# n7koirala/image_matching

Hardware: AMD Instinct MI355X
Metric: encrypted DB vectors matched/sec (HyDia indexScenario, CKKS N=2^15) (higher is better)
Workload: dtype u64

## Files before the change

### image_matching_amd/csrc/context.cpp

```cpp
#include <algorithm>
#include <cmath>
#include <cstdio>
#include <cstdlib>
#include <cstring>

#include <sys/stat.h>

#include "hydia_core.h"

namespace hydia {

u64 mulmod_u64(u64 a, u64 b, u64 q) { return (u64)(((u128)a * b) % q); }
u64 powmod_u64(u64 a, u64 e, u64 q) {
    u64 r = 1 % q;
    a %= q;
    for (; e; e >>= 1) {
        if (e & 1) r = mulmod_u64(r, a, q);
        a = mulmod_u64(a, a, q);
    }
    return r;
}
u64 invmod_u64(u64 a, u64 q) { return powmod_u64(a % q, q - 2, q); }

static bool miller_rabin(u64 n) {
// ... 292 lines not shown
                ifr[2 * i] = (double)itw[i];
                ifr[2 * i + 1] = (double)itw[i] / qd;
            }
        HIP_CHECK(hipMalloc((void **)&d_twf, 2 * tb));
        HIP_CHECK(hipMalloc((void **)&d_itwf, 2 * tb));
        HIP_CHECK(hipMemcpy(d_twf, fr.data(), 2 * tb, hipMemcpyHostToDevice));
        HIP_CHECK(hipMemcpy(d_itwf, ifr.data(), 2 * tb, hipMemcpyHostToDevice));
        std::vector<double> dr((size_t)nT * N), idr((size_t)nT * N);
        for (size_t i = 0; i < (size_t)nT * N; i++) {
            dr[i] = (double)tw[i];
            idr[i] = (double)itw[i];
        }
        HIP_CHECK(hipMalloc((void **)&d_twd, tb));
        HIP_CHECK(hipMalloc((void **)&d_itwd, tb));
        HIP_CHECK(hipMemcpy(d_twd, dr.data(), tb, hipMemcpyHostToDevice));
        HIP_CHECK(hipMemcpy(d_itwd, idr.data(), tb, hipMemcpyHostToDevice));
    }
    tabs = NttTables{d_tw, d_tw_sh, d_itw, d_itw_sh, d_mod, (const ulonglong2 *)d_twp, (const ulonglong2 *)d_itwp,
                     (const ulonglong2 *)d_twf, (const ulonglong2 *)d_itwf, (const double *)d_twd, (const double *)d_itwd, 0u};
    if (getenv("HYDIA_NTT_INT")) tabs.twf = tabs.itwf = nullptr;
    getenv_int_arith = getenv("HYDIA_NTT_INT") != nullptr;
    tabs.fp_mask = 0;
    for (int m = 0; m < nT; m++)
        if (tabs.twf != nullptr && mod[m].ks + 2 <= 47) tabs.fp_mask |= 1u << m;
    {
        const char *sw = getenv("HYDIA_NTT_1PASS");
        tabs.one_pass = !sw ? 0 : (sw[0] == 'p' ? 2 : 1);
        const char *mn = getenv("HYDIA_NTT_1PASS_MIN");
        tabs.one_pass_min = mn ? atoi(mn) : 1024;
        tabs.two_ip_launches = getenv("HYDIA_RELIN_TWO_IP_LAUNCHES") ? 1 : 0;
        tabs.no_drop_in_ip = getenv("HYDIA_NO_DROP_IN_IP") ? 1 : 0;
        tabs.int_epilogue = getenv("HYDIA_INT_EPILOGUE") ? 1 : 0;
        const char *g = getenv("HYDIA_IP_GROUP");
        tabs.ip_group = g && atoi(g) > 0 ? atoi(g) : 8;
        tabs.generic = getenv("HYDIA_NTT_GENERIC") ? 1 : 0;
        tabs.cf_wide = getenv("HYDIA_COLFUSE_WIDE") ? 1 : 0;
        tabs.p2_wg_sync = getenv("HYDIA_P2_WG_SYNC") ? 1 : 0;
        tabs.no_tw_lds = getenv("HYDIA_NO_TW_LDS") ? 1 : 0;
    }
    modup_per_digit = getenv("HYDIA_MODUP_PER_DIGIT") != nullptr;
    loop_a_separate_ip = getenv("HYDIA_LOOPA_SEPARATE_IP") != nullptr;
    loop_a_int_ip = getenv("HYDIA_LOOPA_INT_IP") != nullptr;
    loop_a_limb_fastest = getenv("HYDIA_LOOPA_LIMB_FASTEST") != nullptr;
    relin_separate_intt = getenv("HYDIA_RELIN_SEPARATE_INTT") != nullptr;
    tabs.pm_mask = 0;
    if (!getenv("HYDIA_NTT_INT") && !getenv("HYDIA_NTT_NO_PM"))
        for (int m = 0; m < nT; m++)
            if (!((tabs.fp_mask >> m) & 1u) && mod[m].q < (1ull << 60) && (1ull << 60) - mod[m].q < (1ull << 24)) tabs.pm_mask |= 1u << m;
    if (const char *e = getenv("HYDIA_TENSOR_BPP")) tensor_bpp = std::max(1, atoi(e));
    if (const char *e = getenv("HYDIA_TENSOR_NW")) tensor_nw = atoi(e);
    merge_rescale = getenv("HYDIA_NO_MERGE_RESCALE") == nullptr;
    fuse_ip = getenv("HYDIA_NO_FUSE_IP") == nullptr;
    fork_products = getenv("HYDIA_NO_FORK") == nullptr;
    fuse_loop_a = getenv("HYDIA_NO_FUSE_LOOPA") == nullptr;
    colfuse = getenv("HYDIA_NO_COLFUSE") == nullptr;
    if (const char *e = getenv("HYDIA_MATVEC")) {
        if (e[0] == 'h') matvec_mode = 1;
        else if (e[0] == 'b') matvec_mode = bsgs_babies();
        else if (e[0] >= '1' && e[0] <= '9') matvec_mode = babies_for(1, atoi(e));
        else matvec_mode = 0;
    }
    rot_packed = getenv("HYDIA_KEYS_UNPACKED") == nullptr;
    db_packed = getenv("HYDIA_DB_UNPACKED") == nullptr;
    db_seq_ok = getenv("HYDIA_DB_CT_MAJOR") == nullptr;
    for (int j = 1; j < nQ; j++)
        if (q[j] >> 48) db_packed = false;
    HIP_CHECK(hipMalloc((void **)&d_rotptrs, sizeof(u64 *) * (size_t)p.dim));
    HIP_CHECK(hipMalloc((void **)&d_rotgalois, sizeof(unsigned) * (size_t)p.dim));
    HIP_CHECK(hipMalloc((void **)&d_rotginv, sizeof(unsigned) * (size_t)p.dim));

}

Context::~Context() {
    (void)hipSetDevice(device);
    for (auto st : lane_stream) (void)hipStreamSynchronize(st);
    stream = lane_stream.empty() ? stream : lane_stream[0];
    for (auto &kv : timers)
        for (auto &ev : kv.second.pending) {
            (void)hipEventDestroy(ev.first);
            (void)hipEventDestroy(ev.second);
        }
    pool.trim();
    for (auto &kv : modup_plans)
        if (kv.second.d_tabs) (void)hipFree(kv.second.d_tabs);
    for (auto &kv : cf_plans)
        if (kv.second.dev) (void)hipFree(kv.second.dev);
    rot_keys[0] = relin_key;
    for (auto &kv : rot_keys)
        if (!kv.second.borrowed)
            for (void *p : {(void *)kv.second.d, (void *)kv.second.d_cell, (void *)kv.second.d_gal})
                if (p) (void)hipFree(p);
    if (keys_borrowed) d_rotpack = nullptr, d_sk = nullptr, d_pk = nullptr;
    for (void *p : {(void *)d_mod, (void *)d_tw, (void *)d_tw_sh, (void *)d_itw, (void *)d_itw_sh, (void *)d_twp, (void *)d_itwp, (void *)d_twf, (void *)d_itwf, (void *)d_twd, (void *)d_itwd,
                    (void *)d_rotptrs, (void *)d_rotpack, (void *)d_giant_keys, (void *)d_giant_gal, (void *)d_giant_ginv,
                    (void *)d_rotgalois, (void *)d_rotginv, (void *)d_sk, (void *)d_pk, (void *)d_db, (void *)d_rot_group, (void *)d_ksi})
        if (p) (void)hipFree(p);
    for (auto e : lane_ev) (void)hipEventDestroy(e);
    for (auto e : par_ev)
        if (e) (void)hipEventDestroy(e);
    for (size_t k = 1; k < lane_stream.size(); k++) (void)hipStreamDestroy(lane_stream[k]);
    if (stream) (void)hipStreamDestroy(stream);
}
void Context::set_lane(int k) {
    stream = lane_stream[k];
    pool.cur = k;
}
void Context::sync_all() {
    for (auto st : lane_stream) HIP_CHECK(hipStreamSynchronize(st));
}

LimbSel Context::sel_q(int nl) const { return sel_range(0, nl); }
LimbSel Context::sel_range(int lo, int hi) const {
    LimbSel s{};
    s.n = hi - lo;
    for (int j = lo; j < hi; j++) s.mod[j - lo] = j;
    return s;
}
LimbSel Context::sel_ext(int nl) const {
    LimbSel s{};
    s.n = nl + nP;
    for (int j = 0; j < nl; j++) s.mod[j] = j;
    for (int k = 0; k < nP; k++) s.mod[nl + k] = nQ + k;
    return s;
}
ScaleSel Context::scale_ninv(const LimbSel &s) const {
    ScaleSel r{};
    for (int i = 0; i < s.n; i++) {
        r.s[i] = mod[s.mod[i]].ninv;
        r.s_sh[i] = mod[s.mod[i]].ninv_sh;
    }
    return r;
}
ScaleSel Context::scale_of(const LimbSel &s, const std::vector<u64> &v, bool times_ninv) const {
    ScaleSel r{};
    for (int i = 0; i < s.n; i++) {
        u64 qq = q[s.mod[i]];
        u64 val = v[i] % qq;
        if (times_ninv) val = mulmod_u64(val, mod[s.mod[i]].ninv, qq);
        r.s[i] = val;
        r.s_sh[i] = shoup(val, qq);
    }
    return r;
}
u64 Context::galois_elt(int rot) const {
    u64 M = 2ull * N, g = 1;
    int r = ((rot % slots) + slots) % slots;
    for (int i = 0; i < r; i++) g = (g * 5) % M;
    return g;
}

void Context::adopt_keys(Context &src) {
    if (&src == this) return;
    if (src.device != device) throw std::runtime_error("hydia: keys can only be shared between contexts on the same GPU");
    if (src.nT != nT || src.N != N || src.prm.dnum != prm.dnum || src.prm.dim != prm.dim || src.q != q)
        throw std::runtime_error("hydia: keys can only be shared between contexts with identical parameters");
    if (relin_key.d || !rot_keys.empty() || d_sk || d_pk) throw StateError("hydia: this context already holds keys of its own");
    src.build_rotptrs();
    src.sync_all();
// ... 273 lines not shown
```

### image_matching_amd/csrc/evaluator.cpp

```cpp
#include <algorithm>
#include <cmath>
#include <cstring>

#include "hydia_core.h"

#include <exception>

namespace hydia {

static u64 shoup_h(u64 w, u64 q) { return (u64)(((u128)w << 64) / q); }

static void op_bytes(const char *op, size_t N, double transforms, double other_bytes) {
    hk::ledger_add(op, transforms * 2.0 * (double)N * 8.0 + other_bytes);
}

void Context::ntt_fwd(u64 *base, size_t outer, int X, const LimbSel &s) {
    if (X <= 0 || s.n <= 0) return;
    hk::ntt_forward(stream, tabs, prm.logN, base, base, outer, outer, X, s);
}
void Context::ntt_inv(const u64 *src, u64 *dst, size_t so, size_t dso, int X, const LimbSel &s, const ScaleSel &sc) {
    if (X <= 0 || s.n <= 0) return;
    hk::ntt_inverse(stream, tabs, prm.logN, src, dst, so, dso, X, s, sc);
}

// ... 127 lines not shown
    cf.usc = mod[l].ninv;
    cf.usc_sh = mod[l].ninv_sh;
    for (int k = 0; k < nP; k++) {
        const u64 qq = q[nQ + k];
        cf.smod[k] = nQ + k;
        cf.srow[k] = 1 + k;
        cf.ssc[k] = mulmod_u64(Phat_inv[k] % qq, mod[nQ + k].ninv, qq);
        cf.ssc_sh[k] = shoup_h(cf.ssc[k], qq);
        for (int j = 0; j < nl; j++) {
            u64 f = mulmod_u64(Phat_mod_q[k][j], Pinv_mod_q[j], q[j]);
            if (dbl) f = (f + f) % q[j];
            if (j < l) cf.f[k][j] = f;
            else cf.fl[k] = f;
        }
    }
    for (int j = 0; j < l; j++) {
        cf.tmod[j] = j;
        cf.trow[j] = j;
    }
    return cf_plan_store(key, std::move(maps));
}

const Context::CfPlan &Context::cf_plan_rescale(int nl) {
    const std::string key = "rs:" + std::to_string(nl);
    auto it = cf_plans.find(key);
    if (it != cf_plans.end()) return it->second;
    const int l = nl - 1;
    if (l > HY_CF_TGT) throw std::runtime_error("hydia: too many targets for the column-fused conversion");
    std::vector<ColFuse> maps(1);
    ColFuse &cf = maps[0];
    cf = ColFuse{};
    cf.nk = 0;
    cf.nt = l;
    cf.mdr = 1;
    cf.l = l;
    cf.umod = l;
    cf.urow = 0;
    cf.usc = mod[l].ninv;
    cf.usc_sh = mod[l].ninv_sh;
    for (int j = 0; j < l; j++) {
        cf.tmod[j] = j;
        cf.trow[j] = j;
    }
    return cf_plan_store(key, std::move(maps));
}

void Context::modup_digits(const u64 *c, size_t c_outer, int X, int nl, u64 *dig, bool copy_own, bool p1_only, const ProdSrc *ps, u64 *d2_out) {
    if (ps && !cf_ok()) throw std::runtime_error("hydia: fused product outside the column-fused pipeline");
    const int nE = nl + nP, nd = (nl + alpha - 1) / alpha;
    const size_t dig_x = (size_t)nd * nE * N;
    const LimbSel esel = sel_ext(nl), qsel = sel_q(nl);
    const ModUpPlan &pl = modup_plan(nl);
    u64 *y = pool.get((size_t)X * nl * N * sizeof(u64));
    if (cf_ok()) {
        const CfPlan &cp = cf_plan_modup(nl);
        const bool small = hk::ntt15_colfuse_small(X, nd);
        if (ps) {
            hk::ntt15_inverse_p2_prod(stream, tabs, *ps, y, (size_t)nl * N, X, qsel, d2_out);
            if (small) hk::ntt15_inverse_p1(stream, tabs, y, (size_t)nl * N, X, qsel, scale_of(qsel, pl.inv, true));
        } else if (small) {
            ntt_inv(c, y, c_outer, (size_t)nl * N, X, qsel, scale_of(qsel, pl.inv, true));
        } else {
            hk::ntt15_inverse_p2(stream, tabs, c, y, c_outer, (size_t)nl * N, X, qsel);
        }
        hk::ntt15_colfuse(stream, tabs, y, (size_t)nl * N, dig, dig_x, X, cp.dev, cp.host.data(), nd, small);
        pool.put(y);
        if (!p1_only) {
            if ((size_t)X * nd * nE < 128) {
                hk::ntt15_forward_p2(stream, tabs, dig, (size_t)nE * N, X * nd, esel);
            } else {
                for (int d = 0; d < nd; d++) {
                    const int lo = d * alpha, hi = std::min(lo + alpha, nl);
                    u64 *out = dig + (size_t)d * nE * N;
                    LimbSel rest{};
                    rest.n = nE - hi;
                    for (int t = hi; t < nE; t++) rest.mod[t - hi] = esel.mod[t];
                    if (lo > 0) hk::ntt15_forward_p2(stream, tabs, out, dig_x, X, sel_range(0, lo));
                    if (rest.n > 0) hk::ntt15_forward_p2(stream, tabs, out + (size_t)hi * N, dig_x, X, rest);
                }
            }
        }
        if (copy_own)
            for (int d = 0; d < nd; d++) {
                const int lo = d * alpha, hi = std::min(lo + alpha, nl);
                hk::copy_limbs(stream, N, c + (size_t)lo * N, dig + (size_t)d * nE * N + (size_t)lo * N, c_outer, dig_x, X, hi - lo);
            }
        return;
    }
    ntt_inv(c, y, c_outer, (size_t)nl * N, X, qsel, scale_of(qsel, pl.inv, true));
    hk::base_convert_digits(stream, d_mod, N, y, (size_t)nl * N, dig, dig_x, X, pl.d_tabs, nd, nl, nE, esel);
    const bool merged = !modup_per_digit && nd > 1 && (size_t)X * nd * nE < 128;
    if (merged) {
        if (p1_only) hk::ntt15_forward_p1(stream, tabs, dig, dig, (size_t)nE * N, (size_t)nE * N, X * nd, esel);
        else ntt_fwd(dig, (size_t)nE * N, X * nd, esel);
    }
    for (int d = 0; d < nd; d++) {
        const int lo = d * alpha, hi = std::min(lo + alpha, nl), sz = hi - lo;
        u64 *out = dig + (size_t)d * nE * N;
        LimbSel rest{};
        rest.n = nE - hi;
        for (int t = hi; t < nE; t++) rest.mod[t - hi] = esel.mod[t];
        if (!merged) {
            if (p1_only) {
                if (lo > 0) hk::ntt15_forward_p1(stream, tabs, out, out, dig_x, dig_x, X, sel_range(0, lo));
                if (rest.n > 0) hk::ntt15_forward_p1(stream, tabs, out + (size_t)hi * N, out + (size_t)hi * N, dig_x, dig_x, X, rest);
            } else {
                if (lo > 0) ntt_fwd(out, dig_x, X, sel_range(0, lo));
                ntt_fwd(out + (size_t)hi * N, dig_x, X, rest);
            }
        }
        if (copy_own) hk::copy_limbs(stream, N, c + (size_t)lo * N, out + (size_t)lo * N, c_outer, dig_x, X, sz);
    }
    pool.put(y);
}

void Context::ks_apply(const u64 *dig, size_t dig_x_stride, int X, int nl, const u64 *const *d_keys, int same_key,
                       const u64 *addend, size_t add_x_stride, size_t add_poly_stride, int add_polys,
// ... 203 lines not shown
    pool.put(y);
    std::vector<u64> pinv(Pinv_mod_q.begin(), Pinv_mod_q.begin() + nl);
    NttStore stp{};
    stp.mode = 1;
    stp.out = out;
    stp.nl = nl;
    stp.in = acc;
    stp.in_ls = nE;
    stp.mul = scale_of(qsel, pinv, false);
    stp.addend = addend;
    stp.add_x = add_x;
    stp.add_p = add_p;
    stp.add_polys = add_polys;
    stp.dbl = dbl ? 1 : 0;
    stp.ginv = d_ginv;
    stp.same_g = same_g;
    hk::ntt15_forward_p2_fused(stream, tabs, conv, (size_t)nl * N, XP, qsel, stp);
    pool.put(conv);
    pool.put(acc);
}

void Context::relinearize(Ct &c, bool dbl) {
    if (c.npoly != 3) return;
    if (!relin_key.d) throw StateError("hydia: relinearisation key not loaded");
    const int nl = c.nl, nE = nl + nP, nd = (nl + alpha - 1) / alpha, X = c.X;
    op_bytes("op:relinearize", N, (double)X * (nd * nE + 2 * nP + 2 * nl), (double)nd * 2 * nE * N * 8);
    if (ks_fused_ok()) {
        Ct out(this, X, 2, nl, c.scale);
        ks_fused(c.d + 2 * c.poly_elems(), c.ct_elems(), X, nl, relin_key.d, relin_key.d_cell, nullptr, c.d, c.ct_elems(), c.poly_elems(), 2, nullptr, 0, dbl,
                 out.d);
        c = std::move(out);
        return;
    }
    u64 *dig = pool.get((size_t)X * nd * nE * N * sizeof(u64));
    modup_digits(c.d + 2 * c.poly_elems(), c.ct_elems(), X, nl, dig);
    Ct out(this, X, 2, nl, c.scale);
    ks_apply(dig, (size_t)nd * nE * N, X, nl, relin_key.d_cell, 1, c.d, c.ct_elems(), c.poly_elems(), 2, nullptr, nullptr, 0, dbl,
             out.d);
    pool.put(dig);
    c = std::move(out);
}
void Context::rescale(Ct &c, const Ct *sub, const double *addc) {
    const int nl = c.nl, l = nl - 1, XP = c.X * c.npoly;
    if (nl < 2) throw std::runtime_error("hydia: rescale with one limb left");
    if (sub && (sub->X != c.X || sub->npoly != c.npoly || sub->nl < l)) throw std::runtime_error("hydia: rescale sub operand shape");
    op_bytes("op:rescale", N, (double)XP * nl, 0);
    u64 *t = pool.get((size_t)XP * N * sizeof(u64));
    const LimbSel last = sel_range(l, l + 1);
    u64 *tmp = pool.get((size_t)XP * l * N * sizeof(u64));
    const LimbSel qsel = sel_q(l);
    Ct out(this, c.X, c.npoly, l, c.scale / (double)q[l]);
    std::vector<u64> qi(ql_inv[l].begin(), ql_inv[l].begin() + l);
    const bool rcf = rescale_cf && cf_ok() && l <= HY_LC_LIMBS && l <= HY_CF_TGT && (q[l] >> 50) == 0 && XP >= 256;
    if (rcf) {
        hk::ntt15_inverse_p2(stream, tabs, c.d + (size_t)l * N, t, c.poly_elems(), (size_t)N, XP, last);
        const CfPlan &cp = cf_plan_rescale(nl);
        hk::ntt15_colfuse(stream, tabs, t, (size_t)N, tmp, (size_t)l * N, XP, cp.dev, cp.host.data(), 1, false);
        NttStore stp{};
        stp.mode = 2;
        stp.out = out.d;
        stp.nl = l;
        stp.in = c.d;
        stp.in_ls = c.lstride;
        stp.mul = scale_of(qsel, qi, false);
        stp.sub = sub ? sub->d : nullptr;
        stp.sub_ls = sub ? sub->lstride : 0;
        stp.has_addc = addc ? 1 : 0;
        stp.npoly = c.npoly;
        if (addc)
            for (int j = 0; j < l; j++) stp.addc[j] = double_to_mod(*addc * out.scale, q[j]);
        hk::ntt15_forward_p2_fused(stream, tabs, tmp, (size_t)l * N, XP, qsel, stp);
        pool.put(tmp);
        pool.put(t);
        c = std::move(out);
        return;
    }
    ntt_inv(c.d + (size_t)l * N, t, c.poly_elems(), (size_t)N, XP, last, scale_ninv(last));
    if (prm.logN == 15 && l <= HY_LC_LIMBS) {
        NttLoad ld{};
        ld.mode = 2;
        ld.y = t;
        ld.y_outer = (size_t)N;
        ld.l = l;
        NttStore stp{};
        stp.mode = 2;
        stp.out = out.d;
        stp.nl = l;
        stp.in = c.d;
        stp.in_ls = c.lstride;
        stp.mul = scale_of(qsel, qi, false);
        stp.sub = sub ? sub->d : nullptr;
        stp.sub_ls = sub ? sub->lstride : 0;
        stp.has_addc = addc ? 1 : 0;
        stp.npoly = c.npoly;
        if (addc)
            for (int j = 0; j < l; j++) stp.addc[j] = double_to_mod(*addc * out.scale, q[j]);
        hk::ntt15_forward_fused(stream, tabs, nullptr, tmp, 0, (size_t)l * N, XP, qsel, ld, stp);
    } else {
        hk::rescale_spread(stream, d_mod, N, t, tmp, XP, l);
        ntt_fwd(tmp, (size_t)l * N, XP, qsel);
        hk::rescale_combine(stream, d_mod, N, c.d, tmp, out.d, XP, l, scale_of(qsel, qi, false), c.lstride);
        if (sub) {
            Ct sv = sub->alias(l);
            sub_inplace(out, sv);
        }
        if (addc) add_const(out, *addc);
    }
    pool.put(tmp);
    pool.put(t);
    c = std::move(out);
}
void Context::relin_rescale(Ct &c, bool dbl, const Ct *sub, const double *addc, bool sub_is_add) {
    if (c.npoly != 3) throw std::runtime_error("hydia: relin_rescale needs a 3-component ciphertext");
    const int nl = c.nl, l = nl - 1;
    if (prm.logN != 15 || !merge_rescale || l < 1 || l > HY_LC_LIMBS) {
        relinearize(c, dbl);
        rescale(c, sub_is_add ? nullptr : sub, addc);
        if (sub && sub_is_add) {
            Ct sv = sub->alias(l);
            add_inplace(c, sv);
        }
        return;
    }
    if (!relin_key.d) throw StateError("hydia: relinearisation key not loaded");
    if (sub && (sub->X != c.X || sub->npoly != 2 || sub->nl < l)) throw std::runtime_error("hydia: rescale sub operand shape");
    Ct out(this, c.X, 2, l, c.scale / (double)q[l]);
    relin_rescale_into(c, dbl, sub, addc, sub_is_add, out.d);
    c = std::move(out);
}
void Context::relin_rescale_into(const Ct &c, bool dbl, const Ct *sub, const double *addc, bool sub_is_add, u64 *out_d, const ProdSrc *ps,
                                 const ScaleSel *kap) {
    const int nl = c.nl, l = nl - 1;
    const int nE = nl + nP, nd = (nl + alpha - 1) / alpha, X = c.X, XP = X * 2;
    op_bytes("op:relin_rescale", N, (double)X * (nd * nE + 2 * nP + 4 * nl), (double)nd * 2 * nE * N * 8);
    u64 *dig = pool.get((size_t)X * nd * nE * N * sizeof(u64));
    u64 *d2buf = ps ? pool.get((size_t)X * nl * N * sizeof(u64)) : nullptr;
    const u64 *c2 = ps ? d2buf : c.d + 2 * c.poly_elems();
    const size_t c2_xs = ps ? (size_t)nl * N : c.ct_elems();
    const bool fip = fuse_ip;
    modup_digits(c2, c2_xs, X, nl, dig, false, fip, ps, d2buf);
    const LimbSel esel = sel_ext(nl);
    u64 *acc = pool.get((size_t)XP * nE * N * sizeof(u64));
    const size_t yu_outer = (size_t)(1 + nP) * N;
    u64 *yu = pool.get((size_t)XP * yu_outer * sizeof(u64));
    const bool tail_in_ip = !relin_separate_intt;
    const bool fused_tail = fip && tail_in_ip && prm.logN == 15;
    const LimbSel qsel_full = sel_q(nl);
    std::vector<u64> pinv(Pinv_mod_q.begin(), Pinv_mod_q.begin() + nl);
    const ScaleSel pinv_sel = scale_of(qsel_full, pinv, false);
    const DropLimb drop{l, dbl ? 1 : 0, pinv_sel.s[l], pinv_sel.s_sh[l], c.d, ps ? 0 : c.ct_elems(), ps ? 0 : c.poly_elems(), ps};
    bool drop_done = false;
    timer_begin("ks_inner_product");
    if (fip)
        drop_done = hk::ntt15_p2_inner_product(stream, tabs, d_mod, dig, (size_t)nd * nE * N, nd, X, nl, nP, nT, alpha, relin_key.d_cell, relin_key.d,
                                               c2, c2_xs, acc, fused_tail ? yu : nullptr, yu_outer, 1, fused_tail ? &drop : nullptr);
    else
        hk::inner_product(stream, d_mod, N, dig, (size_t)nd * nE * N, nd, relin_key.d_cell, 1, nT, acc, X, esel, c2, c2_xs, alpha, nl);
    timer_end("ks_inner_product");
    pool.put(dig);
    if (d2buf) pool.put(d2buf);
    if (ps && !(drop_done && fused_tail)) throw std::runtime_error("hydia: fused product outside the merged pipeline (prod_fusable out of step)");
    if (!fused_tail)
        hk::moddown_last_limb(stream, d_mod, N, acc, nE, c.d, c.ct_elems(), c.poly_elems(), acc + (size_t)l * N, (size_t)nE * N, XP, l,
                              pinv_sel.s[l], pinv_sel.s_sh[l], dbl ? 1 : 0);
    LimbSel tail{};
    tail.n = 1 + nP;
    tail.mod[0] = l;
    std::vector<u64> tail_scale(1 + nP, 1);
    for (int k = 0; k < nP; k++) {
        tail.mod[1 + k] = nQ + k;
        tail_scale[1 + k] = Phat_inv[k];
    }
    const bool cfu = cf_ok() && (q[l] >> 50) == 0;
    const bool cf_pre = cfu && cf_small_moddown(XP);
    if (fused_tail) {
        if (!drop_done)
            hk::ntt15_inverse_p2_last_limb(stream, tabs, acc + (size_t)l * N, yu, (size_t)nE * N, yu_outer, XP, l, pinv_sel.s[l], pinv_sel.s_sh[l],
                                           c.d, c.ct_elems(), c.poly_elems(), dbl ? 1 : 0);
        if (!cfu || cf_pre) hk::ntt15_inverse_p1(stream, tabs, yu, yu_outer, XP, tail, scale_of(tail, tail_scale, true));
    } else if (cfu && !cf_pre) {
        hk::ntt15_inverse_p2(stream, tabs, acc + (size_t)l * N, yu, (size_t)nE * N, yu_outer, XP, tail);
    } else {
        ntt_inv(acc + (size_t)l * N, yu, (size_t)nE * N, yu_outer, XP, tail, scale_of(tail, tail_scale, true));
    }
    const u64 *u = yu, *y = yu + N;
    ConvTab tab{};
    tab.ns = nP;
    tab.nt = nl;
    for (int k = 0; k < nP; k++)
        for (int j = 0; j < nl; j++) {
            u64 f = mulmod_u64(Phat_mod_q[k][j], Pinv_mod_q[j], q[j]);
            tab.f[k][j] = dbl ? (f + f) % q[j] : f;
        }
    u64 *w = pool.get((size_t)XP * l * N * sizeof(u64));
    if (cfu) {
        const CfPlan &cp = cf_plan_moddown_rescale(nl, dbl);
        hk::ntt15_colfuse(stream, tabs, yu, yu_outer, w, (size_t)l * N, XP, cp.dev, cp.host.data(), 1, cf_pre);
    } else {
        hk::moddown_rescale_conv(stream, d_mod, N, y, yu_outer, u, yu_outer, w, XP, l, nP, tab);
    }
    const LimbSel qsel = sel_q(l);
    const double out_scale = c.scale / (double)q[l];
    std::vector<u64> qi(ql_inv[l].begin(), ql_inv[l].begin() + l);
    NttLoad ld{};
    NttStore stp{};
    stp.mode = 3;
    stp.out = out_d;
    stp.nl = l;
    stp.in = acc;
    stp.in_ls = nE;
    stp.mul = pinv_sel;
    stp.mul2 = scale_of(qsel, qi, false);
    stp.addend = c.d;
    stp.add_x = ps ? 0 : c.ct_elems();
    stp.add_p = ps ? 0 : c.poly_elems();
    stp.add_polys = 2;
    if (ps) {
        stp.has_prod = 1;
        stp.prod = *ps;
        if (ps->c) stp.kap = *kap;
    }
    stp.dbl = dbl ? 1 : 0;
    stp.sub = sub ? sub->d : nullptr;
    stp.sub_ls = sub ? sub->lstride : 0;
    stp.sub_add = sub_is_add ? 1 : 0;
    stp.has_addc = addc ? 1 : 0;
    stp.npoly = 2;
    if (addc)
        for (int j = 0; j < l; j++) stp.addc[j] = double_to_mod(*addc * out_scale, q[j]);
    if (cfu) hk::ntt15_forward_p2_fused(stream, tabs, w, (size_t)l * N, XP, qsel, stp);
    else hk::ntt15_forward_fused(stream, tabs, w, w, (size_t)l * N, (size_t)l * N, XP, qsel, ld, stp);
    pool.put(w);
    pool.put(yu);
    pool.put(acc);
}
Ct Context::clone(const Ct &a) {
    Ct o(this, a.X, a.npoly, a.nl, a.scale);
    hk::copy_limbs(stream, N, a.d, o.d, a.poly_elems(), o.poly_elems(), a.X * a.npoly, a.nl);
    return o;
}
void Context::drop_to(Ct &a, int nl) {
    if (nl < a.nl) a.nl = nl;
}
static void check_same(const Ct &a, const Ct &b, const char *what) {
    if (a.X != b.X || a.npoly != b.npoly || a.nl != b.nl)
        throw std::runtime_error(std::string("hydia: shape mismatch in ") + what);
}
void Context::add_inplace(Ct &a, const Ct &b) {
    check_same(a, b, "add");
    op_bytes("op:add", N, 0, 3.0 * a.X * a.npoly * a.nl * N * 8);
    hk::add(stream, d_mod, N, a.d, b.d, a.d, a.X * a.npoly, sel_q(a.nl), a.lstride, b.lstride, a.lstride);
}
void Context::sub_inplace(Ct &a, const Ct &b) {
    check_same(a, b, "sub");
    op_bytes("op:add", N, 0, 3.0 * a.X * a.npoly * a.nl * N * 8);
    hk::sub(stream, d_mod, N, a.d, b.d, a.d, a.X * a.npoly, sel_q(a.nl), a.lstride, b.lstride, a.lstride);
}
void Context::add_const(Ct &a, double c) {
    const LimbSel s = sel_q(a.nl);
    ScaleSel sc{};
    for (int j = 0; j < a.nl; j++) sc.s[j] = double_to_mod(c * a.scale, q[j]);
    hk::add_scalar(stream, d_mod, N, a.d, a.ct_elems(), a.X, s, sc);
}
Ct Context::mul_const(const Ct &a, double c, double const_scale) {
    const LimbSel s = sel_q(a.nl);
    ScaleSel sc{};
    for (int j = 0; j < a.nl; j++) {
        sc.s[j] = double_to_mod(c * const_scale, q[j]);
        sc.s_sh[j] = shoup_h(sc.s[j], q[j]);
    }
    Ct o(this, a.X, a.npoly, a.nl, a.scale * const_scale);
    hk::mul_scalar(stream, d_mod, N, a.d, o.d, a.X * a.npoly, s, sc, a.lstride, o.lstride);
    return o;
}
Ct Context::lincomb(const std::vector<const Ct *> &terms, const std::vector<double> &coef, double c0, double S) {
    if (terms.empty() || terms.size() > HY_LC_TERMS || terms.size() != coef.size()) throw std::runtime_error("hydia: bad lincomb");
    const Ct &f = *terms[0];
    if (f.nl > HY_LC_LIMBS) throw std::runtime_error("hydia: lincomb limb count");
    LinComb lc{};
    lc.nterms = (int)terms.size();
    for (int t = 0; t < lc.nterms; t++) {
        const Ct &a = *terms[t];
        if (a.X != f.X || a.npoly != f.npoly || a.nl != f.nl) throw std::runtime_error("hydia: lincomb shape mismatch");
        lc.src[t] = a.d;
        lc.ls[t] = a.lstride;
        for (int j = 0; j < f.nl; j++) {
            lc.c[t][j] = double_to_mod(coef[t] * (S / a.scale), q[j]);
            lc.cs[t][j] = shoup_h(lc.c[t][j], q[j]);
        }
    }
    for (int j = 0; j < f.nl; j++) lc.c0[j] = double_to_mod(c0 * S, q[j]);
    op_bytes("op:lincomb", N, 0, (double)(lc.nterms + 1) * f.X * f.npoly * f.nl * N * 8);
    Ct o(this, f.X, f.npoly, f.nl, S);
    hk::lincomb(stream, d_mod, N, lc, o.d, f.X, f.npoly, f.nl);
    return o;
}
Ct Context::lincomb_multi(const std::vector<const Ct *> &terms, const std::vector<std::vector<double>> &coef,
                          const std::vector<double> &c0, const std::vector<double> &S) {
    const int K = (int)coef.size(), nt = (int)terms.size();
    if (nt < 1 || nt > HY_LC_TERMS || K < 1 || (int)c0.size() != K || (int)S.size() != K) throw std::runtime_error("hydia: bad lincomb_multi");
    const Ct &f = *terms[0];
    if (f.nl > HY_LC_LIMBS) throw std::runtime_error("hydia: lincomb limb count");
    LinCombMulti lc{};
    lc.nterms = nt;
    lc.K = K;
    lc.fp = (tabs.twf != nullptr || prm.logN != 15) && !getenv_int_arith ? 1 : 0;
    if (lcm_stage.size() >= 64) {
        sync_all();
        lcm_stage.clear();
    }
    lcm_stage.emplace_back((size_t)K * HY_LCM_BLOCK, 0);
    std::vector<u64> &lcm_host = lcm_stage.back();
    for (int t = 0; t < nt; t++) {
        const Ct &a = *terms[t];
        if (a.X != f.X || a.npoly != f.npoly || a.nl != f.nl) throw std::runtime_error("hydia: lincomb shape mismatch");
        lc.src[t] = a.d;
        lc.ls[t] = a.lstride;
        for (int k = 0; k < K; k++)
            for (int j = 0; j < f.nl; j++)
                lcm_host[(size_t)k * HY_LCM_BLOCK + t * HY_LC_LIMBS + j] = double_to_mod(coef[k][t] * (S[k] / a.scale), q[j]);
    }
    for (int k = 0; k < K; k++)
        for (int j = 0; j < f.nl; j++) lcm_host[(size_t)k * HY_LCM_BLOCK + HY_LC_TERMS * HY_LC_LIMBS + j] = double_to_mod(c0[k] * S[k], q[j]);
    u64 *tab = pool.get(lcm_host.size() * sizeof(u64));
    HIP_CHECK(hipMemcpyAsync(tab, lcm_host.data(), lcm_host.size() * sizeof(u64), hipMemcpyHostToDevice, stream));
    lc.tab = tab;
    op_bytes("op:lincomb", N, 0, (double)(nt + K) * f.X * f.npoly * f.nl * N * 8);
    Ct o(this, f.X * K, f.npoly, f.nl, S[0]);
    hk::lincomb_multi(stream, d_mod, N, lc, o.d, f.X, f.npoly, f.nl);
    pool.put(tab);
    return o;
}
Ct Context::mult_norelin(const Ct &a, const Ct &b) {
    if (a.X != b.X || a.nl != b.nl || a.npoly != 2 || b.npoly != 2) throw std::runtime_error("hydia: mult shape mismatch");
    op_bytes("op:mult_norelin", N, 0, 7.0 * a.X * a.nl * N * 8);
    Ct o(this, a.X, 3, a.nl, a.scale * b.scale);
    hk::tensor(stream, d_mod, N, a.d, b.d, o.d, a.X, a.nl, a.lstride, b.lstride);
    return o;
}
Ct Context::mult_norelin_sub(const Ct &a, const Ct &b, const Ct &c) {
    if (a.X != b.X || a.nl != b.nl || a.npoly != 2 || b.npoly != 2 || c.X != a.X || c.npoly != 2 || c.nl != a.nl)
        throw std::runtime_error("hydia: mult-sub shape mismatch");
    op_bytes("op:mult_norelin", N, 0, 9.0 * a.X * a.nl * N * 8);
    Ct o(this, a.X, 3, a.nl, a.scale * b.scale);
    const u64 K = (u64)std::llround(o.scale / c.scale);
    ScaleSel kap{};
    for (int j = 0; j < a.nl; j++) {
        const u64 inv2 = (q[j] + 1) >> 1;
        kap.s[j] = mulmod_u64(K % q[j], inv2, q[j]);
        kap.s_sh[j] = shoup_h(kap.s[j], q[j]);
    }
    hk::tensor(stream, d_mod, N, a.d, b.d, o.d, a.X, a.nl, a.lstride, b.lstride, c.d, c.lstride, &kap);
    return o;
}
bool Context::prod_fusable(int nl) const {
    const int l = nl - 1, nd = (nl + alpha - 1) / alpha;
    return prod_fuse && prm.logN == 15 && merge_rescale && fuse_ip && !relin_separate_intt && cf_ok() && l >= 1 && l <= HY_LC_LIMBS && nd >= 2 &&
           nd <= 4 && !tabs.two_ip_launches && !tabs.no_drop_in_ip && (q[l] >> 50) == 0 && relin_key.d != nullptr;
}
Ct Context::mult_relin_rescale(const Ct &a, const Ct &b, bool dbl, const Ct *sub, const double *addc, bool sub_is_add, const Ct *csub) {
    if (a.X != b.X || a.nl != b.nl || a.npoly != 2 || b.npoly != 2) throw std::runtime_error("hydia: mult shape mismatch");
    if (csub && (csub->X != a.X || csub->npoly != 2 || csub->nl != a.nl || !dbl)) throw std::runtime_error("hydia: mult-sub shape mismatch");
    if (csub && sub) throw std::logic_error("hydia: mult_relin_rescale takes a product subtrahend (csub) or a sub operand, not both");
    const int nl = a.nl, l = nl - 1, nd = (nl + alpha - 1) / alpha;
    if (!prod_fusable(nl) || (csub && (!prod_fuse_csub || nd < 3)) || (sub && (sub->X != a.X || sub->npoly != 2 || sub->nl < l))) {
        Ct o = csub ? mult_norelin_sub(a, b, *csub) : mult_norelin(a, b);
        relin_rescale(o, dbl, sub, addc, sub_is_add);
        return o;
    }
    op_bytes("op:mult_norelin", N, 0, (csub ? 9.0 : 7.0) * a.X * a.nl * N * 8);
    Ct shape;
    shape.ctx = this;
    shape.X = a.X;
    shape.npoly = 3;
    shape.nl = shape.lstride = nl;
    shape.scale = a.scale * b.scale;
    shape.view = true;
    ProdSrc ps{a.d, b.d, a.ct_elems(), a.poly_elems(), b.ct_elems(), b.poly_elems(), nullptr, 0, 0, 0, 0};
    ScaleSel kap{};
    if (csub) {
        const u64 K = (u64)std::llround(shape.scale / csub->scale);
        for (int j = 0; j < nl; j++) {
            const u64 inv2 = (q[j] + 1) >> 1;
            kap.s[j] = mulmod_u64(K % q[j], inv2, q[j]);
            kap.s_sh[j] = shoup_h(kap.s[j], q[j]);
        }
        ps.c = csub->d;
        ps.c_x = csub->ct_elems();
        ps.c_p = csub->poly_elems();
        ps.kap_l = kap.s[l];
        ps.kap_l_sh = kap.s_sh[l];
    }
    Ct out(this, a.X, 2, l, shape.scale / (double)q[l]);
    relin_rescale_into(shape, dbl, sub, addc, sub_is_add, out.d, &ps, &kap);
    return out;
}
Ct Context::mult(const Ct &a, const Ct &b) {
    const int nl = std::min(a.nl, b.nl);
    Ct x = a.alias(nl), y = b.alias(nl);
    return mult_relin_rescale(x, y);
}
Ct Context::rotate(const Ct &a, int rot) {
    auto it = rot_keys.find(rot);
    if (it == rot_keys.end()) throw StateError("hydia: rotation key " + std::to_string(rot) + " not loaded");
// ... 367 lines not shown
             if (degree >= 8) {
                 ch.G.push_back(ch.T[8].alias(ch.T[8].nl));
                 gi = 0;
                 while ((8 << (gi + 1)) <= degree) {
                     Ct nx = cheb_step(this, ch.G[gi], ch.G[gi], nullptr);
                     ch.G.push_back(std::move(nx));
                     gi++;
                 }
             }
         });
    Ct y = cheb_combine(ch, tr);
    tr.groups.clear();
    ch.G.clear();
    ch.T.clear();
    Ct y2 = mult(y, y), y3, y4, y8;
    par2([&] { y3 = mult(y2, y); }, [&] { y4 = mult(y2, y2); });
    const int nl = y3.nl;
    Ct yd = y.alias(nl);
    const int y8_nl = y4.nl - 1;
    const double y8_scale = (y4.scale * y4.scale) / (double)q[y4.nl - 1];
    Ct v, u, w;
    double a_scale = 0;
    par2([&] {
             v = lincomb({&yd, &y3}, {F4[5], F4[7]}, 0.0, delta * (double)q[nl - 1]);
             rescale(v);
             v.scale = delta;
             a_scale = (v.scale * y4.scale) / (double)q[std::min(v.nl, y4.nl) - 1];
             u = lincomb({&yd, &y3}, {F4[1], F4[3]}, 0.0, a_scale * (double)q[nl - 1]);
             rescale(u);
             u.scale = a_scale;
             const int lb = std::min(y.nl - 1, y8_nl);
             const double wt = a_scale * (double)q[lb - 1] / y8_scale;
             w = lincomb({&y}, {F4[9]}, 0.0, wt * (double)q[y.nl - 1]);
             rescale(w);
             w.scale = wt;
         },
         [&] { y8 = mult(y4, y4); });
    if (y8.nl != y8_nl || y8.scale != y8_scale) throw std::runtime_error("hydia: comparator scale plan out of step");
    Ct au = mult_add(this, v, y4, u);
    Ct a = mult_add(this, w, y8, au);
    a.scale = a_scale;
    add_const(a, 1.0);
    return a;
}

Ct Context::relin_compare_lanes(Ct &acc, double dlt, int sign_depth) {
    const int G = acc.X, L = std::min(nlanes, G);
    const bool relin = acc.npoly == 3;
    if (L <= 1) {
        if (relin) relin_rescale(acc);
        else rescale(acc);
        return chebyshev_compare(acc, dlt, sign_depth);
    }
    while ((int)lane_ev.size() < nlanes + 1) {
        hipEvent_t e;
        HIP_CHECK(hipEventCreateWithFlags(&e, hipEventDisableTiming));
        lane_ev.push_back(e);
    }
    std::vector<hipEvent_t> &ev = lane_ev;
    struct LaneGuard {
        Context *c;
        ~LaneGuard() {
            c->set_lane(0);
            c->side_lane_free = true;
            if (std::uncaught_exceptions() > 0)
                for (auto st : c->lane_stream) (void)hipStreamSynchronize(st);
        }
    } guard{this};
    side_lane_free = false;
    HIP_CHECK(hipEventRecord(ev[L], stream));
    std::vector<Ct> res(L);
    Ct out;
    for (int k = 0; k < L; k++) {
        const int g0 = (int)((long)G * k / L), g1 = (int)((long)G * (k + 1) / L);
        set_lane(k);
        if (k > 0) HIP_CHECK(hipStreamWaitEvent(stream, ev[L], 0));
        Ct part = acc.alias(acc.nl);
        part.X = g1 - g0;
        part.d = acc.d + (size_t)g0 * acc.ct_elems();
        if (relin) relin_rescale(part);
        else rescale(part);
        res[k] = chebyshev_compare(part, dlt, sign_depth);
        if (k == 0) {
            out = Ct(this, G, res[0].npoly, res[0].nl, res[0].scale);
            HIP_CHECK(hipEventRecord(ev[0], stream));
        } else {
            HIP_CHECK(hipStreamWaitEvent(stream, ev[0], 0));
        }
        Ct rk = res[k].compact() ? res[k].alias(res[k].nl) : clone(res[k]);
        HIP_CHECK(hipMemcpyAsync(out.d + (size_t)g0 * out.ct_elems(), rk.d, rk.bytes(), hipMemcpyDeviceToDevice, stream));
        if (k > 0) HIP_CHECK(hipEventRecord(ev[k], stream));
    }
    set_lane(0);
    for (int k = 1; k < L; k++) HIP_CHECK(hipStreamWaitEvent(stream, ev[k], 0));
    res.clear();
    return out;
}
Ct Context::similarity_accumulate(const Ct &qc) {
    if (!d_db || db_cts == 0 || db_kind != 5) throw StateError("hydia: no database resident (diagonal packing)");
    if (qc.nl != nQ) throw StateError("hydia: query must be a fresh (level 0) ciphertext");
    Ct rot = rotate_query(qc);
    return similarity_accumulate_rot(rot);
}
Ct Context::similarity_accumulate_rot(const Ct &rot) {
    if (!d_db || db_cts == 0 || db_kind != 5) throw StateError("hydia: no database resident (diagonal packing)");
    const int dim = prm.dim;
    if (rot.X != dim || rot.npoly != 2 || rot.nl != nQ || !rot.compact())
        throw StateError("hydia: rotations must be vector_dim fresh 2-component ciphertexts");
    const int G = (int)(db_cts / dim);
    Ct acc(this, G, 3, nQ, rot.scale * delta);
    op_bytes("op:loop_b", N, 0, (double)db_cts * (double)db_layout().ct_bytes + ((double)dim * 2 + (double)G * 3) * nQ * N * 8);
    timer_begin("hydia_tensor");
    hk::hydia_tensor_accumulate(stream, d_mod, N, rot.d, 0, d_db, acc.d, 1, G, dim, nQ, db_lay, 0, tensor_bpp, tensor_nw);
    timer_end("hydia_tensor");
    return acc;
}
Ct Context::similarity_rot(const Ct &rot) {
    Ct acc = similarity_accumulate_rot(rot);
    relin_rescale(acc);
    return acc;
}
Ct Context::index_scenario_rot(const Ct &rot) {
    Ct acc = similarity_accumulate_rot(rot);
    return relin_compare_lanes(acc, 0.44, 10);
}
Ct Context::index_scenario(const Ct &qc) {
    Ct acc = db_kind == 6 ? similarity_bsgs_sum(qc) : similarity_accumulate(qc);
    return relin_compare_lanes(acc, 0.44 , 10 );
}
// ... 150 lines not shown
```

### image_matching_amd/csrc/hydia_core.h

```cpp
#pragma once
#include <hip/hip_runtime.h>

#include <cstdint>
#include <exception>
#include <map>
#include <mutex>
#include <memory>
#include <stdexcept>
#include <string>
#include <vector>

#include "kernels.h"

namespace hydia {
struct DeviceError : std::runtime_error {
    using std::runtime_error::runtime_error;
};
struct StateError : std::runtime_error {
    using std::runtime_error::runtime_error;
};
}

#define HIP_CHECK(expr)                                                                                   \
    do {                                                                                                  \
// ... 22 lines not shown
  private:
    std::recursive_mutex mu_;
    std::map<int, std::multimap<size_t, u64 *>> free_;
    std::map<u64 *, std::pair<size_t, int>> size_;
};

struct Context;

struct Ct {
    Context *ctx = nullptr;
    u64 *d = nullptr;
    int X = 0, npoly = 0, nl = 0, lstride = 0;
    double scale = 0;
    bool view = false;
    Ct() = default;
    Ct(Context *c, int X_, int npoly_, int nl_, double scale_);
    Ct(const Ct &) = delete;
    Ct &operator=(const Ct &) = delete;
    Ct(Ct &&o) noexcept { *this = std::move(o); }
    Ct &operator=(Ct &&o) noexcept;
    ~Ct();
    size_t poly_elems() const;
    size_t ct_elems() const { return (size_t)npoly * poly_elems(); }
    size_t bytes() const { return ct_elems() * X * sizeof(u64); }
    bool compact() const { return lstride == nl; }
    Ct alias(int nl_) const;
};

struct KernelTimer {
    double total_ms = 0;
    long launches = 0;
    std::vector<std::pair<hipEvent_t, hipEvent_t>> pending;
};

struct HostParams {
    Params prm;
    int N, slots, nQ, nP, nT, alpha;
    double delta;
    std::vector<u64> q, psi;
    std::vector<ModC> mod;
    std::vector<u64> P_mod_q, Pinv_mod_q, Phat_inv;
    std::vector<std::vector<u64>> Phat_mod_q;
    std::vector<std::vector<u64>> ql_inv;
    explicit HostParams(const Params &p);
    void twiddles(int m, std::vector<u64> &tw, std::vector<u64> &tws, std::vector<u64> &itw, std::vector<u64> &itws) const;
};

struct Context : HostParams {
    int device;
    hipStream_t stream = nullptr;
    std::vector<hipStream_t> lane_stream;
    int nlanes = 2;
    std::vector<hipEvent_t> lane_ev;
    void set_lane(int k);
    void sync_all();
    template <class F0, class F1>
    void par2(F0 &&here, F1 &&side);
    bool side_lane_free = true;
    hipEvent_t par_ev[2] = {nullptr, nullptr};
    Pool pool;

    ModC *d_mod = nullptr;
    u64 *d_tw = nullptr, *d_tw_sh = nullptr, *d_itw = nullptr, *d_itw_sh = nullptr, *d_twp = nullptr, *d_itwp = nullptr, *d_twf = nullptr, *d_itwf = nullptr, *d_twd = nullptr, *d_itwd = nullptr;
    NttTables tabs{};

    struct EvalKey {
        u64 *d = nullptr;
        const u64 **d_cell = nullptr;
        unsigned *d_gal = nullptr;
        bool borrowed = false;
    };
    EvalKey relin_key;
    std::map<int, EvalKey> rot_keys;
    const u64 **d_rotptrs = nullptr;
    unsigned *d_rotgalois = nullptr;
    unsigned *d_rotginv = nullptr;
    bool rotptrs_valid = false, rotptrs_packed = false, rotptrs_premul = false;
    unsigned char *d_rotpack = nullptr;
    bool rot_packed = true;
    void adopt_keys(Context &src);
    bool keys_borrowed = false;
    void load_eval_key(int rot , const u64 *host);
    u64 *eval_key_storage(int rot);
    u64 *d_sk = nullptr;
    u64 *d_pk = nullptr;
    unsigned *d_rot_group = nullptr;
    double *d_ksi = nullptr;

    unsigned char *d_db = nullptr;
    size_t db_vectors = 0, db_cts = 0;
    int db_kind = 0;
    int db_babies = 0;
    int matvec_mode = 0;
    int bsgs_babies() const {
        int B = 1;
        while (B * B < prm.dim) B <<= 1;
        return B;
    }
    int auto_babies(size_t blocks) const {
        const int base = bsgs_babies();
        static const struct { size_t limit; int mult; } rule[] = {{3, 2}, {12, 4}, {40, 8}};
        for (const auto &r : rule)
            if (blocks <= r.limit) return std::min(prm.dim, base * r.mult);
        return prm.dim;
    }
    int babies_for(size_t blocks, int explicit_mode = 0) const {
// ... 185 lines not shown
```

Before: 20.20 million.

## Stagger second lane start to offset kernel phases between parallel streams

```diff
diff --git a/image_matching_amd/csrc/context.cpp b/image_matching_amd/csrc/context.cpp
--- a/image_matching_amd/csrc/context.cpp
+++ b/image_matching_amd/csrc/context.cpp
@@ -368,6 +368,7 @@
     merge_rescale = getenv("HYDIA_NO_MERGE_RESCALE") == nullptr;
     fuse_ip = getenv("HYDIA_NO_FUSE_IP") == nullptr;
     fork_products = getenv("HYDIA_NO_FORK") == nullptr;
+    lanes_in_step = getenv("HYDIA_LANES_IN_STEP") != nullptr;
     fuse_loop_a = getenv("HYDIA_NO_FUSE_LOOPA") == nullptr;
     colfuse = getenv("HYDIA_NO_COLFUSE") == nullptr;
     if (const char *e = getenv("HYDIA_MATVEC")) {
@@ -420,6 +421,10 @@
 void Context::set_lane(int k) {
     stream = lane_stream[k];
     pool.cur = k;
+}
+void Context::seam_release() {
+    HIP_CHECK(hipEventRecord(lane_ev.back(), stream));
+    seam_released = true;
 }
 void Context::sync_all() {
     for (auto st : lane_stream) HIP_CHECK(hipStreamSynchronize(st));
diff --git a/image_matching_amd/csrc/evaluator.cpp b/image_matching_amd/csrc/evaluator.cpp
--- a/image_matching_amd/csrc/evaluator.cpp
+++ b/image_matching_amd/csrc/evaluator.cpp
@@ -203,6 +203,7 @@
     const LimbSel esel = sel_ext(nl), qsel = sel_q(nl);
     const ModUpPlan &pl = modup_plan(nl);
     u64 *y = pool.get((size_t)X * nl * N * sizeof(u64));
+    seam();
     if (cf_ok()) {
         const CfPlan &cp = cf_plan_modup(nl);
         const bool small = hk::ntt15_colfuse_small(X, nd);
@@ -214,6 +215,7 @@
         } else {
             hk::ntt15_inverse_p2(stream, tabs, c, y, c_outer, (size_t)nl * N, X, qsel);
         }
+        seam();
         hk::ntt15_colfuse(stream, tabs, y, (size_t)nl * N, dig, dig_x, X, cp.dev, cp.host.data(), nd, small);
         pool.put(y);
         if (!p1_only) {
@@ -523,9 +525,11 @@
     Ct out(this, c.X, c.npoly, l, c.scale / (double)q[l]);
     std::vector<u64> qi(ql_inv[l].begin(), ql_inv[l].begin() + l);
     const bool rcf = rescale_cf && cf_ok() && l <= HY_LC_LIMBS && l <= HY_CF_TGT && (q[l] >> 50) == 0 && XP >= 256;
+    seam();
     if (rcf) {
         hk::ntt15_inverse_p2(stream, tabs, c.d + (size_t)l * N, t, c.poly_elems(), (size_t)N, XP, last);
         const CfPlan &cp = cf_plan_rescale(nl);
+        seam();
         hk::ntt15_colfuse(stream, tabs, t, (size_t)N, tmp, (size_t)l * N, XP, cp.dev, cp.host.data(), 1, false);
         NttStore stp{};
         stp.mode = 2;
@@ -540,6 +544,7 @@
         stp.npoly = c.npoly;
         if (addc)
             for (int j = 0; j < l; j++) stp.addc[j] = double_to_mod(*addc * out.scale, q[j]);
+        seam();
         hk::ntt15_forward_p2_fused(stream, tabs, tmp, (size_t)l * N, XP, qsel, stp);
         pool.put(tmp);
         pool.put(t);
@@ -566,6 +571,7 @@
         stp.npoly = c.npoly;
         if (addc)
             for (int j = 0; j < l; j++) stp.addc[j] = double_to_mod(*addc * out.scale, q[j]);
+        seam();
         hk::ntt15_forward_fused(stream, tabs, nullptr, tmp, 0, (size_t)l * N, XP, qsel, ld, stp);
     } else {
         hk::rescale_spread(stream, d_mod, N, t, tmp, XP, l);
@@ -621,6 +627,7 @@
     const ScaleSel pinv_sel = scale_of(qsel_full, pinv, false);
     const DropLimb drop{l, dbl ? 1 : 0, pinv_sel.s[l], pinv_sel.s_sh[l], c.d, ps ? 0 : c.ct_elems(), ps ? 0 : c.poly_elems(), ps};
     bool drop_done = false;
+    seam();
     timer_begin("ks_inner_product");
     if (fip)
         drop_done = hk::ntt15_p2_inner_product(stream, tabs, d_mod, dig, (size_t)nd * nE * N, nd, X, nl, nP, nT, alpha, relin_key.d_cell, relin_key.d,
@@ -664,6 +671,7 @@
             tab.f[k][j] = dbl ? (f + f) % q[j] : f;
         }
     u64 *w = pool.get((size_t)XP * l * N * sizeof(u64));
+    seam();
     if (cfu) {
         const CfPlan &cp = cf_plan_moddown_rescale(nl, dbl);
         hk::ntt15_colfuse(stream, tabs, yu, yu_outer, w, (size_t)l * N, XP, cp.dev, cp.host.data(), 1, cf_pre);
@@ -699,6 +707,7 @@
     stp.npoly = 2;
     if (addc)
         for (int j = 0; j < l; j++) stp.addc[j] = double_to_mod(*addc * out_scale, q[j]);
+    seam();
     if (cfu) hk::ntt15_forward_p2_fused(stream, tabs, w, (size_t)l * N, XP, qsel, stp);
     else hk::ntt15_forward_fused(stream, tabs, w, w, (size_t)l * N, (size_t)l * N, XP, qsel, ld, stp);
     pool.put(w);
@@ -763,6 +772,7 @@
     for (int j = 0; j < f.nl; j++) lc.c0[j] = double_to_mod(c0 * S, q[j]);
     op_bytes("op:lincomb", N, 0, (double)(lc.nterms + 1) * f.X * f.npoly * f.nl * N * 8);
     Ct o(this, f.X, f.npoly, f.nl, S);
+    seam();
     hk::lincomb(stream, d_mod, N, lc, o.d, f.X, f.npoly, f.nl);
     return o;
 }
@@ -798,6 +808,7 @@
     lc.tab = tab;
     op_bytes("op:lincomb", N, 0, (double)(nt + K) * f.X * f.npoly * f.nl * N * 8);
     Ct o(this, f.X * K, f.npoly, f.nl, S[0]);
+    seam();
     hk::lincomb_multi(stream, d_mod, N, lc, o.d, f.X, f.npoly, f.nl);
     pool.put(tab);
     return o;
@@ -806,6 +817,7 @@
     if (a.X != b.X || a.nl != b.nl || a.npoly != 2 || b.npoly != 2) throw std::runtime_error("hydia: mult shape mismatch");
     op_bytes("op:mult_norelin", N, 0, 7.0 * a.X * a.nl * N * 8);
     Ct o(this, a.X, 3, a.nl, a.scale * b.scale);
+    seam();
     hk::tensor(stream, d_mod, N, a.d, b.d, o.d, a.X, a.nl, a.lstride, b.lstride);
     return o;
 }
@@ -821,6 +833,7 @@
         kap.s[j] = mulmod_u64(K % q[j], inv2, q[j]);
         kap.s_sh[j] = shoup_h(kap.s[j], q[j]);
     }
+    seam();
     hk::tensor(stream, d_mod, N, a.d, b.d, o.d, a.X, a.nl, a.lstride, b.lstride, c.d, c.lstride, &kap);
     return o;
 }
@@ -1294,7 +1307,7 @@
         else rescale(acc);
         return chebyshev_compare(acc, dlt, sign_depth);
     }
-    while ((int)lane_ev.size() < nlanes + 1) {
+    while ((int)lane_ev.size() < nlanes + 2) {
         hipEvent_t e;
         HIP_CHECK(hipEventCreateWithFlags(&e, hipEventDisableTiming));
         lane_ev.push_back(e);
@@ -1305,18 +1318,24 @@
         ~LaneGuard() {
             c->set_lane(0);
             c->side_lane_free = true;
+            c->seam_countdown = -1;
             if (std::uncaught_exceptions() > 0)
                 for (auto st : c->lane_stream) (void)hipStreamSynchronize(st);
         }
     } guard{this};
     side_lane_free = false;
     HIP_CHECK(hipEventRecord(ev[L], stream));
+    seam_countdown = (L == 2 && !lanes_in_step) ? phase_shift : -1;
+    seam_released = false;
     std::vector<Ct> res(L);
     Ct out;
     for (int k = 0; k < L; k++) {
         const int g0 = (int)((long)G * k / L), g1 = (int)((long)G * (k + 1) / L);
         set_lane(k);
-        if (k > 0) HIP_CHECK(hipStreamWaitEvent(stream, ev[L], 0));
+        if (k > 0) {
+            seam_countdown = -1;
+            HIP_CHECK(hipStreamWaitEvent(stream, seam_released ? ev.back() : ev[L], 0));
+        }
         Ct part = acc.alias(acc.nl);
         part.X = g1 - g0;
         part.d = acc.d + (size_t)g0 * acc.ct_elems();
diff --git a/image_matching_amd/csrc/hydia_core.h b/image_matching_amd/csrc/hydia_core.h
--- a/image_matching_amd/csrc/hydia_core.h
+++ b/image_matching_amd/csrc/hydia_core.h
@@ -98,6 +98,14 @@
     std::vector<hipStream_t> lane_stream;
     int nlanes = 2;
     std::vector<hipEvent_t> lane_ev;
+    static constexpr int phase_shift = 2;
+    int seam_countdown = -1;
+    bool seam_released = false;
+    bool lanes_in_step = false;
+    void seam() {
+        if (seam_countdown >= 0 && seam_countdown-- == 0) seam_release();
+    }
+    void seam_release();
     void set_lane(int k);
     void sync_all();
     template <class F0, class F1>
```

Result: no change. 20.21 million (median of 3 runs) (+0.1%).
